# getreu/stringsext

Measured on AMD Instinct MI355X. Metric: GiB/s scanned, higher is better.
Workload: dtype u8

## Files before the change

### stringsext_amd/csrc/sx_device.hpp

```cpp
#pragma once
#include <cstdlib>
#include <hip/hip_runtime_api.h>
#include <stdint.h>

#include "../../include/stringsext_amd.h"

namespace sx {

constexpr uint32_t kTileBytes = 1024;

struct DevRun {
    uint64_t start;
    uint32_t len;
    uint32_t chars_flags;
};
constexpr uint32_t kRecStartOpen = 0x80000000u;
constexpr uint32_t kRecEndOpen = 0x40000000u;
constexpr uint32_t kRecCharsMask = 0x3FFFFFFFu;
constexpr uint32_t kRecInvalidLen = 0xFFFFFFFFu, kRecInvalidFlags = 0xFFFFFFFFu;

constexpr uint32_t kStatBase = 32, kStatShards = 16, kStatStride = 32, kCounterWords = kStatBase + kStatShards * kStatStride;

enum ClassifierKind : uint32_t {
    kClsSingleByteLut = 0,
// ... 76 lines not shown
struct ReplayRegionOut {
    uint64_t end;
    uint32_t n_find, n_bytes, status, pad;
};
size_t replay_heads_scratch_bytes(uint64_t n_runs);
hipError_t launch_replay_heads(const ReplayParams& P, uint32_t* slot_of, uint32_t* n_heads, uint32_t* head_list, ReplayRegionOut* ro,
                               void* scratch, size_t scratch_bytes,
                               hipStream_t stream);
hipError_t launch_replay_count(const ReplayParams& P, ReplayRegionOut* out, hipStream_t stream, int count_waves);
bool replay_fast_covers(const ReplayParams& P);
hipError_t launch_replay_fast(const ReplayParams& P, ReplayRegionOut* out, hipStream_t stream);
hipError_t launch_replay_write(const ReplayParams& P, const uint64_t* region_index, const uint64_t* fbase,
                               const uint64_t* abase, uint64_t n_regions, sx_finding* findings, uint8_t* arena,
                               hipStream_t stream);

size_t split_scratch_bytes(uint64_t n_runs);
hipError_t launch_split_count(const ReplayParams& P, void* scratch, size_t scratch_bytes, uint64_t* d_total, hipStream_t stream);
hipError_t launch_split_write(const ReplayParams& P, const void* scratch, uint64_t n_pieces, sx_run* out, hipStream_t stream);

inline uint32_t stitch_block_runs(uint64_t n_runs, int block_override) {
    if (block_override > 0) return (uint32_t)block_override;
    return n_runs > (1ull << 20) ? 512u : 128u;
}
enum : uint32_t { kTotEnd = 0, kTotLast, kTotFindings, kTotBytes, kTotStanding, kTotReplayBytes, kTotTooLong, kTotLastStart, kTotCount };
size_t stitch_scratch_bytes(uint64_t n_runs);
size_t stitch_blocks_bytes(uint64_t n_runs, int block_override);
hipError_t launch_stitch_blocks(const ReplayParams& P, const ReplayRegionOut* ro, uint8_t* stands, void* blocks,
                                uint64_t* totals, hipStream_t stream, int block_override);
hipError_t launch_stitch_finish(const ReplayParams& P, const ReplayRegionOut* ro, uint8_t* stands, const void* blocks,
                                uint64_t E0, uint64_t* fpos, uint64_t* apos, uint64_t* totals, void* scratch,
                                size_t scratch_bytes, hipStream_t stream, int block_override);
hipError_t launch_replay_write_flagged(const ReplayParams& P, const ReplayRegionOut* ro, const uint8_t* stands,
                                       const uint64_t* fpos, const uint64_t* apos, sx_finding* findings,
                                       uint8_t* arena, uint64_t avg_out_bytes, hipStream_t stream);

struct WvSwar {
    uint32_t cls;
    uint32_t n;
    uint32_t c1[6], c2[6], hi[6];
    uint32_t hi_len;
    uint32_t lr_c1[2], lr_c2[2];
    uint32_t kana;
};
struct WaveParams {
    const uint8_t* data;
    uint64_t len;
    uint64_t consumed0;
    uint32_t slice_base;
    uint32_t W, wps, q, n_min;
    uint64_t g_lo, g_hi;
    uint32_t nwin;
    uint32_t inject;
    int32_t mission_id, file_id;
    uint32_t family;
    const uint8_t* lut;
    const uint16_t* table;
    const uint32_t* pairs;
    uint32_t encoding;
    uint32_t entry_skip;
    uint32_t *wave_nf, *wave_nb, *wave_in, *wave_out;
    uint32_t* wave_grid;
    const uint64_t *wave_fbase, *wave_abase;
    uint64_t f_sub, a_sub;
    sx_finding* findings;
    uint8_t* arena;
    uint32_t packed;
    uint32_t str_off_base;
    uint64_t v0, v1;
    uint32_t* desc;
    uint32_t desc_cap;
    WvSwar swar;
    const uint32_t* pairs2;
    uint64_t* lead_set;
    uint64_t ubf;
    int32_t grep_char;
    uint32_t redo, use_entry;
    uint32_t same;
};
size_t wave_scratch_bytes(uint64_t n_waves);
hipError_t launch_wave_count(const WaveParams& P, uint64_t v0, uint64_t v1, uint64_t* fbase, uint64_t* abase, uint64_t* totals,
                             void* scratch, size_t scratch_bytes, hipStream_t stream);
hipError_t launch_wave_write(const WaveParams& P, uint64_t v0, uint64_t v1, hipStream_t stream);
hipError_t launch_wave_emit(const WaveParams& P, uint64_t v0, uint64_t v1, hipStream_t stream);

hipError_t merge_findings_device_part(const sx_finding* const* f, const uint8_t* const* a, const uint64_t* nf, const uint64_t* nb,
                                      const uint32_t* off0, int n_missions, void* out, void* scratch, size_t scratch_bytes,
                                      hipStream_t stream, int packed = 0, int ordered = 0);
bool merge_part_can_pack(uint64_t n, int n_missions);
hipError_t launch_slab_cuts(const ReplayParams& P, uint32_t n_slabs, uint64_t* idx, uint64_t* hi, hipStream_t stream);
hipError_t launch_merge_cuts(const sx_finding* f, uint64_t n, uint64_t nb, const uint64_t* cuts, uint32_t n_cuts, uint64_t* idx,
                             uint64_t* off, hipStream_t stream);
size_t merge_findings_scratch_bytes(uint64_t n_findings, int n_missions, int ordered = 0);
inline size_t up256(size_t v) { return (v + 255) / 256 * 256; }
size_t order_strings_scratch_bytes(uint64_t n);
hipError_t order_part_strings(void* recs, uint64_t n, int packed, const uint64_t* src, uint8_t* arena, void* scratch, size_t scratch_bytes,
                              hipStream_t stream);
struct PrintParams;
size_t print_scratch_bytes(uint64_t n);
hipError_t print_measure(const PrintParams& P, void* scratch, size_t scratch_bytes, hipStream_t stream, const uint64_t** wbase, const uint64_t** total);
hipError_t print_write(const PrintParams& P, hipStream_t stream);
struct SelectParams;
struct SelsetDevice;
struct SelreDevice;
struct LabelPick;
struct SelectBy {
    enum Kind { kPatterns, kSet, kRegex, kLabels } kind = kPatterns;
    union {
        const SelsetDevice* set = nullptr;
        const SelreDevice* re;
        const LabelPick* pick;
    };
};
size_t select_scratch_bytes(uint64_t n);
hipError_t selset_launch_match(const SelectParams& P, const SelsetDevice& set, uint64_t waves, hipStream_t stream);
hipError_t selre_launch_match(const SelectParams& P, const SelreDevice& re, uint64_t waves, hipStream_t stream);
hipError_t label_launch_pick(const SelectParams& P, const LabelPick& pick, uint64_t waves, hipStream_t stream);
hipError_t select_measure(SelectParams* P, const SelectBy& by, void* scratch, size_t scratch_bytes, hipStream_t stream, const uint32_t** count, const uint64_t** bytes);
size_t select_place_scratch_bytes(uint64_t n_sel);
hipError_t select_place(const SelectParams& P, void* out_recs, uint64_t n_sel, uint8_t* out_arena, void* scratch, size_t scratch_bytes, hipStream_t stream);
struct ExtractParams;
size_t extract_scratch_bytes(uint64_t n);
hipError_t extract_measure(ExtractParams* P, void* scratch, size_t scratch_bytes, hipStream_t stream, const uint64_t** count, const uint64_t** bytes);
size_t extract_place_scratch_bytes(uint64_t n_out);
hipError_t extract_place(const ExtractParams& P, void* out_recs, uint64_t n_out, uint8_t* out_arena, void* scratch, size_t scratch_bytes, hipStream_t stream);
struct SeltallyParams;
hipError_t seltally_launch(const SeltallyParams& P, hipStream_t stream);
struct LabelParams;
hipError_t label_launch(const LabelParams& P, hipStream_t stream);
hipError_t launch_copy_bytes(void* dst, const void* src, uint64_t bytes, uint32_t workgroups, hipStream_t stream, int threads, bool nontemporal);
hipError_t launch_small_copy(void* pinned_dst, const void* dev_src, size_t bytes, hipStream_t stream);

size_t sort_scratch_bytes(uint32_t n);
hipError_t sort_records(DevRun* recs, uint32_t n, uint64_t max_key, void* scratch, size_t scratch_bytes, hipStream_t stream, bool timing);

size_t compact_scratch_bytes(uint64_t n_regions);
hipError_t invalidate_region_slack(DevRun* recs, const uint32_t* counts, uint64_t n_regions, uint32_t region_cap, hipStream_t stream);
hipError_t compact_regions(const DevRun* recs, const uint32_t* counts, uint64_t n_regions, uint32_t region_cap, DevRun* out,
                           uint32_t* total, void* scratch, size_t scratch_bytes, hipStream_t stream);

size_t merge_scratch_bytes(uint32_t n);
hipError_t merge_sorted_records(const DevRun* recs, uint32_t n, uint64_t min_chars, void* scratch, size_t scratch_bytes,
                                sx_run* out, uint32_t* out_count, hipStream_t stream);

hipError_t launch_scan(ClassifierKind kind, const ScanParams& p, hipStream_t stream);
constexpr int kFusedMax = 3;
struct FusedParams {
    ScanParams m[kFusedMax];
    const uint8_t* data;
    uint64_t len;
    uint32_t subchunk;
    uint32_t fsh[kFusedMax][4];
    uint32_t cand_f[kFusedMax];
    uint32_t pf_zero[kFusedMax];
};
int fused_slot_of(ClassifierKind kind, const ScanParams& p);
hipError_t launch_scan_fused(const FusedParams& fp, uint32_t used, hipStream_t stream, int prefilter_override);
hipError_t launch_fill_background(uint8_t* dst, uint64_t first_index, uint64_t len, uint64_t seed,
                                  hipStream_t stream);
hipError_t launch_read_sum(const uint8_t* src, uint64_t len, uint64_t* out, hipStream_t stream, uint32_t subchunk = 0, uint32_t rot = 0);
hipError_t launch_gather(const uint8_t* src, uint8_t* dst, const uint64_t* seg_src, const uint64_t* seg_dst,
                         const uint32_t* seg_len, uint32_t n, hipStream_t stream);

}
```

### stringsext_amd/csrc/sx_fused.hip

```cpp
#include "sx_scan_core.hpp"

namespace sx {

struct NoCls {};

SX_DEV u32 shr1_keep(u32 v, u32 old) { return __builtin_amdgcn_update_dpp(old, v, 0x138, 0xF, 0xF, false); }
SX_DEV u32 ror1(u32 v) { return __builtin_amdgcn_mov_dpp(v, 0x13C, 0xF, 0xF, false); }

static_assert(offsetof(FusedParams, m) == 0, "late_params addresses m[slot] from the start of the kernel-argument segment");
typedef const __attribute__((address_space(4))) ScanParams* KArgMission;
SX_DEV KArgMission late_params(u32 slot) {
    asm volatile("" : "+s"(slot));
    return (KArgMission)__builtin_amdgcn_kernarg_segment_ptr() + slot;
}

struct LateEmitter {
    u32 slot, wave;
    u32 rcount, heavy_n;
    SX_DEV void append(bool want, u64 start, u64 end, u32 chars, u32 flags) {
        const u64 m = __ballot(want);
        if (m == 0) return;
        const KArgMission mp = late_params(slot);
        const u32 cap = mp->region_cap;
        DevRun* const recs = mp->recs;
        const u32 k = rcount + (u32)__popcll(m & ((1ull << lane_id()) - 1ull));
        rcount += (u32)__popcll(m);
        if (want && k < cap) {
            DevRun r;
            r.start = start;
            r.len = (u32)(end - start);
            r.chars_flags = (chars > kRecCharsMask ? kRecCharsMask : chars) | flags;
            recs[wave * cap + k] = r;
        }
    }
    SX_DEV void end_region() {
        const KArgMission mp = late_params(slot);
        const u32 cap = mp->region_cap;
        u32* const counters = mp->counters;
        u32* const shard = counters + kStatBase + (wave & (kStatShards - 1u)) * kStatStride;
        if (lane_id() == 0) {
            if (heavy_n) atomicAdd(shard, heavy_n);
            mp->region_counts[wave] = rcount < cap ? rcount : cap;
            if (rcount) atomicAdd(shard + 1, rcount);
            if (rcount > cap) {
                atomicAdd(counters, rcount - cap);
                atomicMax(counters + 3, rcount);
            }
        }
    }
};

template <class CLS>
struct Prefilter {
    static constexpr bool kHas = false;
    SX_DEV void init(u32) {}
    template <int MODE> SX_DEV bool hit(u32x4) const { return true; }
    SX_DEV bool last_unit_may_pass(u32, u32) const { return true; }
    static int mode_for(const ScanParams&) { return 0; }
    static u32 zero_bits(const ScanParams&) { return 0; }
};
template <int BE_T, int ODD_T>
struct Prefilter<Utf16RangeT<BE_T, ODD_T>> {
    static_assert(BE_T >= 0 && ODD_T >= 0, "the fused kernel knows byte order and parity at compile time");
    static constexpr bool kHas = true;
    u32 zz;
    static u32 zero_bits(const ScanParams& p) {
        u32 top = 0;
        if (p.a_lo <= p.a_hi) top = p.a_hi;
        if (p.u_lo <= p.u_hi && p.u_hi > top) top = p.u_hi;
        u32 mh = top >> 8;
        mh |= mh >> 1; mh |= mh >> 2; mh |= mh >> 4;
        return 0xFFu & ~mh;
    }
    SX_DEV void init(u32 z) { zz = (BE_T ^ ODD_T) ? z * 0x00010001u : z * 0x01000100u; }
    static int mode_for(const ScanParams& p) { return zero_bits(p) == 0u ? 0 : p.min_chars >= 7u ? 1 : p.min_chars >= 3u ? 2 : 0; }
    template <int MODE> SX_DEV bool hit(u32x4 x) const {
        if (MODE == 1) {
            const u32 q0 = __builtin_amdgcn_bitop3_b32(x.x, zz, x.y, 0xC8), q1 = __builtin_amdgcn_bitop3_b32(x.z, zz, x.w, 0xC8);
            return (q0 < q1 ? q0 : q1) == 0u;
        }
        const u32 a = x.x & zz, b = x.y & zz, c = x.z & zz, d = x.w & zz;
        const u32 ab = a < b ? a : b, cd = c < d ? c : d;
        return (ab < cd ? ab : cd) == 0u;
    }
    SX_DEV bool last_unit_may_pass(u32 prev_w, u32 cur_x) const {
        const u32 z8 = (zz | (zz >> 8)) & 0xFFu;
        const u32 hi = BE_T == ODD_T ? prev_w >> 24 : (BE_T ? prev_w >> 16 : cur_x);
        return (hi & z8) == 0u;
    }
};

template <class T, class = void> struct has_classify_g : std::false_type {};
template <class T> struct has_classify_g<T, std::void_t<decltype(std::declval<const T&>().classify_g(u32x4{}, 0u))>> : std::true_type {};
template <class CLS>
SX_DEV u32 classify_fast(const CLS& c, u32x4 x, u32 nx) {
    if constexpr (has_classify_g<CLS>::value) return c.classify_g(x, nx);
    else return c.template classify<false>(x, nx, 32u, false);
}

template <class T, class = void> struct has_starts_from_good : std::false_type {};
template <class T> struct has_starts_from_good<T, std::void_t<decltype(T::kStartsFromGood)>> : std::true_type {};

constexpr u32 kUnknown = 0x80000000u;

template <class CLS, int PFM, int SLOT>
struct Slot {
    static constexpr bool kUsed = !std::is_same<CLS, NoCls>::value;
    static constexpr u32 kSlot = SLOT;
    using PF = Prefilter<CLS>;
    static constexpr bool kPf = PFM != 0 && PF::kHas;
    static constexpr int kPfMode = PFM;
    CLS cls;
    PF pf;
    Carry c;
    LateEmitter em;
    u32 E;
    u32 gtmp, pgtmp, rtmp;
    u32 sh0, sh1, sh2, sh3;
};

template <class C0, class C1, class C2, int PFM>
__global__ __launch_bounds__(256) __attribute__((amdgpu_waves_per_eu(PFM ? 6 : 5))) void scan_kernel_fused(const FusedParams fp) {
    const u32 lane = lane_id();
    Slot<C0, PFM, 0> s0; Slot<C1, PFM, 1> s1; Slot<C2, PFM, 2> s2;

    const u32 wave = blockIdx.x * 4u + uniform(threadIdx.x >> 6);
    const u64 len = fp.len;
    const u64 sub_start = (u64)wave * (u64)fp.subchunk;
    if (sub_start >= len) return;
    const u64 sub_end = (sub_start + fp.subchunk < len) ? sub_start + fp.subchunk : len;

    auto make_cls = [&](auto& cls, u32 slot) {
        using CLS = std::decay_t<decltype(cls)>;
        if constexpr (!std::is_same<CLS, NoCls>::value) {
            const KArgMission mp = late_params(slot);
            ScanParams q;
            q.a_lo = mp->a_lo; q.a_hi = mp->a_hi; q.u_lo = mp->u_lo; q.u_hi = mp->u_hi; q.l3_lo = mp->l3_lo; q.l3_hi = mp->l3_hi;
            q.parity = mp->parity; q.big_endian = mp->big_endian; q.high_all = mp->high_all;
            cls.init(q, nullptr);
        }
    };
    auto setup = [&](auto& S) {
        using ST = std::decay_t<decltype(S)>;
        if constexpr (ST::kUsed) {
            constexpr u32 slot = ST::kSlot;
            if constexpr (ST::kPf) S.pf.init(fp.pf_zero[slot]);
            else make_cls(S.cls, slot);
            S.sh0 = fp.fsh[slot][0]; S.sh1 = fp.fsh[slot][1]; S.sh2 = fp.fsh[slot][2]; S.sh3 = fp.fsh[slot][3];
            S.em.slot = slot; S.em.wave = wave; S.em.rcount = 0; S.em.heavy_n = 0;
            S.c.g63 = 0; S.c.tracked = 0; S.c.t_chars = 0; S.c.t_flags = 0; S.c.t_start = 0;
            S.E = 0; S.gtmp = 0; S.pgtmp = 0; S.rtmp = 0;
        }
    };
    setup(s0); setup(s1); setup(s2);

    const bool has_pre = sub_start >= kTileBytes;
    const u64 win_lo = has_pre ? sub_start - kTileBytes : 0;
    u64 win_hi = sub_end + 2 * kTileBytes;
    if (win_hi > len) win_hi = len;
    const uint8_t* base_ptr = fp.data + win_lo;
    const u32 base_lo = uniform((u32)(uintptr_t)base_ptr), base_hi = uniform((u32)((uintptr_t)base_ptr >> 32));
    const __amdgpu_buffer_rsrc_t rsrc = __builtin_amdgcn_make_buffer_rsrc(
        (void*)(((u64)base_hi << 32) | base_lo), 0, (int)uniform(((u32)(win_hi - win_lo) + 15u) & ~15u), 0x00020000);
    auto load = [&](u32 off) -> u32x4 { return __builtin_amdgcn_raw_buffer_load_b128(rsrc, (int)off, 0, 0); };
    struct TileRegs { u32x4 d; u32 e; };
    auto fetch = [&](u32 off) -> TileRegs {
        TileRegs r;
        const u32 a = off + lane * 16u;
        r.d = load(a);
        r.e = __builtin_amdgcn_raw_buffer_load_b32(rsrc, (int)(a + 16u), 0, 0);
        return r;
    };

    const int n_tiles = (int)((sub_end - sub_start + kTileBytes - 1) / kTileBytes);
    int n_safe = n_tiles;
    while (n_safe > 0 && sub_start + (u64)n_safe * kTileBytes + 16 > len) n_safe--;

    int t = has_pre ? -1 : 0;
    u32 toff = 0;
    TileRegs R0 = fetch(0u), R1 = fetch(kTileBytes), R2;

    auto avail_at = [&](u64 tile_base) -> u32 {
        const u64 b = tile_base + 16ull * lane;
        return b >= len ? 0u : (len - b > 32 ? 32u : (u32)(len - b));
    };
    auto starts_before = [&](const auto& cls, u32 off, u64 tile_base) -> u32 {
        if (off < 16u) return 0u;
        asm volatile("" : "+s"(off));
        const u32x4 x = load(off - 16u);
        const u32 nx = __builtin_amdgcn_raw_buffer_load_b32(rsrc, (int)off, 0, 0);
        const u64 b = tile_base - 16;
        const u32 avail = b >= len ? 0u : (len - b > 32 ? 32u : (u32)(len - b));
        return uniform(cls.template classify<true>(x, nx, avail, true));
    };
    auto context_before = [&](const auto& cls, u32 off, u64 tile_base) -> u32 {
        if (off < kTileBytes) return 0u;
        u32 o = off - kTileBytes;
        asm volatile("" : "+s"(o));
        const TileRegs P = fetch(o);
        const u32 g = cls.template classify<false>(P.d, P.e, avail_at(tile_base - kTileBytes), true);
        const u32 pg = from_prev(g, 0u);
        const u32 gf = (g & 0xFFFFu) | (pg >> 16);
        return bcast(gf | (g & 0xFFFF0000u), 63);
    };

    auto generic_slot = [&](auto& S, const TileRegs& X, u64 tile_base, u32 avail, bool ne, bool have_g) {
        using ST = std::decay_t<decltype(S)>;
        if constexpr (ST::kUsed) {
            constexpr u32 slot = ST::kSlot;
            using CLS = std::decay_t<decltype(S.cls)>;
            CLS local;
            const CLS* cls = &S.cls;
            if constexpr (ST::kPf) {
                const u32 open = S.c.tracked | (S.c.g63 & 0x8000u) | ((S.c.g63 == kUnknown && t == 0) ? 1u : 0u);
                if (t < 0 || (__ballot(S.pf.template hit<ST::kPfMode>(X.d)) == 0 && open == 0u)) { S.c.g63 = kUnknown; return; }
                make_cls(local, slot);
                cls = &local;
                if (S.c.g63 == kUnknown) S.c.g63 = context_before(local, toff, tile_base);
            } else {
                S.c.g63 = bcast(have_g ? S.pgtmp : S.E, 0);
            }
            const KArgMission mp = late_params(slot);
            const u32x4 cur = X.d;
            const u32 g63_in = S.c.g63;
            const bool tracked_in = S.c.tracked != 0;
            const bool fast_g = have_g && !ST::kPf;
            const u32 g = fast_g ? S.gtmp : cls->template classify<false>(cur, X.e, avail, ne);
            const u32 pg = fast_g ? S.pgtmp : from_prev(g, g63_in);
            const u32 gf = (g & 0xFFFFu) | (pg >> 16);
            const u32 g63_out = bcast(gf | (g & 0xFFFF0000u), 63);
            u32 w = (g << 16) | pg;
            u32 r = w;
            if (fast_g) r = S.rtmp;
            else { r &= r << S.sh0; r &= r << S.sh1; r = r & (r << S.sh2) & (r << S.sh3); }
            const bool any_cand = __ballot((r & 0xFFFF0000u) != 0) != 0;
            const bool first_tile = t == 0;
            const bool first_open = first_tile && (g63_in & 0x8000u);
            if (t < 0 || (!any_cand && !tracked_in && !first_open)) {
                S.c.g63 = g63_out;
            } else {
                const u32 min_chars = mp->min_chars;
                const u64 lane_base = tile_base + 16ull * lane;
                u32 s;
                if constexpr (has_starts_from_good<CLS>::value) s = ne ? cls->template classify<true>(cur, X.e, avail, true) : cls->starts_from_good(cur, gf);
                else s = cls->template classify<true>(cur, X.e, avail, ne);
                w = (gf << 16) | (from_prev(gf, g63_in) & 0xFFFFu);
                const u32 s63 = (g63_in & 0x8000u) ? starts_before(*cls, toff, tile_base) : 0u;
                const u32 sw = (s << 16) | (from_prev(s, s63) & 0xFFFFu);
                bool done = false;
                if (!tracked_in && !first_open) done = light_path(w, sw, r, lane_base, S.em, min_chars);
                if (done) S.c.g63 = g63_out;
                else {
                    S.em.heavy_n++;
                    const u64 tile_end = tile_base + kTileBytes < sub_end ? tile_base + kTileBytes : sub_end;
                    heavy_path(gf, s, g, g63_in, s63, r >> 16, tile_base, tile_end, S.c, S.em, min_chars, fp.cand_f[slot], first_tile);
                }
            }
            if constexpr (!ST::kPf) S.E = S.c.g63;
        }
    };
    auto generic_tile = [&](const TileRegs& X, u32 which, bool have_g) {
        const u64 tile_base = sub_start + (u64)((long long)t * (long long)kTileBytes);
        const bool ne = t >= n_safe;
        const u32 avail = ne ? avail_at(tile_base) : 32u;
        if (which & 1u) generic_slot(s0, X, tile_base, avail, ne, have_g);
        if (which & 2u) generic_slot(s1, X, tile_base, avail, ne, have_g);
        if (which & 4u) generic_slot(s2, X, tile_base, avail, ne, have_g);
        toff += kTileBytes; t++;
    };

    auto fast_slot = [&](auto& S, const TileRegs& X, const TileRegs& Zp, bool zprev) -> bool {
        using ST = std::decay_t<decltype(S)>;
        if constexpr (!ST::kUsed) return true;
        else if constexpr (ST::kPf) {
            const u32 open = S.c.tracked | (S.c.g63 & 0x8000u);
            if ((__ballot(S.pf.template hit<ST::kPfMode>(X.d)) | (u64)open) != 0) {
                if (S.c.g63 == kUnknown && zprev && !S.pf.last_unit_may_pass(bcast(Zp.d.w, 63), bcast(X.d.x, 0))) S.c.g63 = 0;
                return false;
            }
            S.c.g63 = kUnknown;
            return true;
        } else {
            const u32 g = classify_fast(S.cls, X.d, X.e);
            const u32 pg = shr1_keep(g, S.E);
            const u32 w = (g << 16) | pg;
            u32 r = w;
            r &= r << S.sh0; r &= r << S.sh1; r = r & (r << S.sh2) & (r << S.sh3);
            S.gtmp = g; S.pgtmp = pg; S.rtmp = r;
            S.E = ror1(g);
            return (__ballot((r & 0xFFFF0000u) != 0) | (u64)S.c.tracked) == 0;
        }
    };
    auto fast_tile = [&](const TileRegs& X, TileRegs& Z, bool zprev) -> u32 {
        u32 zero = 0, one = 1, two = 2;
        asm volatile("" : "+s"(zero), "+s"(one), "+s"(two));
        u32 slow = fast_slot(s1, X, Z, zprev) ? zero : two;
        if (!fast_slot(s2, X, Z, zprev)) slow |= 4u;
        Z = fetch(toff + 2 * kTileBytes);
        slow |= fast_slot(s0, X, Z, false) ? zero : one;
        if (slow == 0) { toff += kTileBytes; t++; }
        return slow;
    };
    constexpr u32 kAll = (Slot<C0, PFM, 0>::kUsed ? 1u : 0u) | (Slot<C1, PFM, 1>::kUsed ? 2u : 0u) | (Slot<C2, PFM, 2>::kUsed ? 4u : 0u);

    for (;;) {
        while (t < n_tiles && (t <= 0 || t + 3 > n_safe)) {
            R2 = fetch(toff + 2 * kTileBytes);
            generic_tile(R0, kAll, false);
            R0 = R1; R1 = R2;
        }
        if (t >= n_tiles) break;
        bool zprev = false;
        do {
            u32 slow;
            if ((slow = fast_tile(R0, R2, zprev)) != 0) generic_tile(R0, slow, true);
            if ((slow = fast_tile(R1, R0, true)) != 0) generic_tile(R1, slow, true);
            if ((slow = fast_tile(R2, R1, true)) != 0) generic_tile(R2, slow, true);
            zprev = true;
        } while (t + 3 <= n_safe);
    }

    auto finish = [&](auto& S) {
        using ST = std::decay_t<decltype(S)>;
        if constexpr (ST::kUsed) {
            constexpr u32 slot = ST::kSlot;
            using CLS = std::decay_t<decltype(S.cls)>;
            const u64 after = sub_start + (u64)n_tiles * kTileBytes;
            CLS local;
            const CLS* cls = &S.cls;
            if constexpr (ST::kPf) {
                make_cls(local, slot);
                cls = &local;
                if (S.c.g63 == kUnknown) S.c.g63 = context_before(local, toff, after);
            } else S.c.g63 = bcast(S.E, 0);
            if (S.c.tracked || (S.c.g63 & 0x8000u)) {
                u64 os; u32 och, ofl;
                if (S.c.tracked) { os = S.c.t_start; och = S.c.t_chars; ofl = S.c.t_flags; }
                else {
                    const u32 suf = trailing_ones16(S.c.g63 & 0xFFFFu);
                    const u32 s63 = starts_before(*cls, toff, after);
                    os = after - suf;
                    och = (u32)__popc((s63 & 0xFFFFu) >> (16u - suf));
                    ofl = 0;
                }
                S.em.append(lane == 0, os, sub_end, och, ofl | kRecEndOpen);
            }
            S.em.end_region();
        }
    };
    finish(s0); finish(s1); finish(s2);
}

template <class C0, class C1, class C2>
static hipError_t launch_f(const FusedParams& fp, uint32_t used, hipStream_t stream, int prefilter_override) {
    const u64 waves = (fp.len + fp.subchunk - 1) / fp.subchunk;
    const u64 blocks = (waves + 3) / 4;
    if (blocks == 0) return hipSuccess;
    FusedParams q = fp;
    int mode = 1;
    if ((used & 2u) && Prefilter<C1>::mode_for(fp.m[1]) != 1) mode = Prefilter<C1>::mode_for(fp.m[1]);
    if ((used & 4u) && mode && Prefilter<C2>::mode_for(fp.m[2]) != 1) mode = Prefilter<C2>::mode_for(fp.m[2]) == 0 ? 0 : 2;
    if (!(used & 6u)) mode = 0;
    if (prefilter_override == 0) mode = 0; else if (prefilter_override == 2 && mode == 1) mode = 2;
    q.pf_zero[0] = 0; q.pf_zero[1] = Prefilter<C1>::zero_bits(fp.m[1]); q.pf_zero[2] = Prefilter<C2>::zero_bits(fp.m[2]);
    if (mode == 1) hipLaunchKernelGGL((scan_kernel_fused<C0, C1, C2, 1>), dim3((unsigned)blocks), dim3(256), 0, stream, q);
    else if (mode == 2) hipLaunchKernelGGL((scan_kernel_fused<C0, C1, C2, 2>), dim3((unsigned)blocks), dim3(256), 0, stream, q);
    else hipLaunchKernelGGL((scan_kernel_fused<C0, C1, C2, 0>), dim3((unsigned)blocks), dim3(256), 0, stream, q);
    return hipGetLastError();
}

int fused_slot_of(ClassifierKind kind, const ScanParams& p) {
    if (p.region_cap == 0 || p.persistent) return -1;
    if (kind == kClsUtf8Range2) return 0;
    if (kind == kClsUtf16Range) return p.big_endian ? 2 : 1;
    return -1;
}

hipError_t launch_scan_fused(const FusedParams& fp, uint32_t used, hipStream_t stream, int prefilter_override) {
    u32 parity = 0;
    if (used & 2u) parity = fp.m[1].parity & 1u; else if (used & 4u) parity = fp.m[2].parity & 1u;
    FusedParams q = fp;
    for (int s = 0; s < kFusedMax; s++) {
        if (!((used >> s) & 1u)) continue;
        q.data = fp.m[s].data; q.len = fp.m[s].len; q.subchunk = fp.m[s].subchunk;
        const u32 c = std::min<u32>(fp.m[s].cand_bytes, 12u);
        q.cand_f[s] = c;
        u32 have = 1;
        const u32 sh0 = have < c ? 1u : 0u; have += sh0;
        const u32 sh1 = have < c ? std::min(have, c - have) : 0u; have += sh1;
        const u32 rem = c - have;
        const u32 sh2 = std::min(have, rem), sh3 = rem;
        q.fsh[s][0] = sh0; q.fsh[s][1] = sh1; q.fsh[s][2] = sh2; q.fsh[s][3] = sh3;
    }
#define SX_ARG(...) __VA_ARGS__
#define SX_F(U, P, A, B, C) if (used == U && parity == P) return launch_f<A, B, C>(q, used, stream, prefilter_override);
    SX_F(1u, 0u, Utf8Range2, NoCls, NoCls)
    SX_F(7u, 0u, Utf8Range2, SX_ARG(Utf16RangeT<0, 0>), SX_ARG(Utf16RangeT<1, 0>))
    SX_F(7u, 1u, Utf8Range2, SX_ARG(Utf16RangeT<0, 1>), SX_ARG(Utf16RangeT<1, 1>))
    SX_F(3u, 0u, Utf8Range2, SX_ARG(Utf16RangeT<0, 0>), NoCls)
    SX_F(3u, 1u, Utf8Range2, SX_ARG(Utf16RangeT<0, 1>), NoCls)
    SX_F(5u, 0u, Utf8Range2, NoCls, SX_ARG(Utf16RangeT<1, 0>))
    SX_F(5u, 1u, Utf8Range2, NoCls, SX_ARG(Utf16RangeT<1, 1>))
    SX_F(6u, 0u, NoCls, SX_ARG(Utf16RangeT<0, 0>), SX_ARG(Utf16RangeT<1, 0>))
    SX_F(6u, 1u, NoCls, SX_ARG(Utf16RangeT<0, 1>), SX_ARG(Utf16RangeT<1, 1>))
#undef SX_F
#undef SX_ARG
    return hipErrorInvalidValue;
}

}
```

### stringsext_amd/csrc/sx_stage_a.cpp

```cpp
#include "sx_ctx.hpp"

using namespace sx;

namespace sx {

static bool large_regions_fit(uint64_t len, uint64_t n_regions, uint32_t cap) {
    const uint64_t slots = n_regions * cap;
    return slots < (1ull << 31) && slots * sizeof(DevRun) <= std::max<uint64_t>(256ull << 20, len / 2);
}

static uint32_t subchunk_bytes(const sx_ctx* ctx) {
    const uint32_t sub = ctx->opt.subchunk_bytes ? ctx->opt.subchunk_bytes : 256u * 1024u;
    return std::max<uint32_t>(kTileBytes, sub / kTileBytes * kTileBytes);
}

static bool fusion_allowed(const sx_ctx* ctx) {
    return !(ctx->opt.flags & (SX_OPT_NO_FUSED_SCAN | SX_OPT_MISSION_STREAMS)) && !ctx->sw.mission_streams && ctx->sw.fused && ctx->sw.scan_warm < 0;
}

ScanParams scan_params(const sx_ctx* ctx, int mission, const ScanSlot& s, const uint8_t* d_bytes, uint64_t len,
                       uint32_t parity, uint64_t min_chars) {
    const Mission& m = ctx->missions[(size_t)mission];
    ScanParams p = m.proto;
    p.data = d_bytes; p.len = len; p.subchunk = subchunk_bytes(ctx); p.parity = parity;
    p.pair_lut = ctx->dev[(size_t)mission].d_pair_lut;
    if (p.gb4) {
        p.gb_ranges = ctx->dev[(size_t)mission].d_table ? ctx->dev[(size_t)mission].d_table + kGbN : nullptr;
        p.ubf = m.c.ubf;
        if (!p.gb_ranges) p.gb4 = 0;
    }
    p.wave_prio = ctx->sw.scan_prio;
    p.min_chars = (uint32_t)std::min<uint64_t>(min_chars, kRecCharsMask);
    if (p.min_chars == 0) p.min_chars = 1;
    p.cand_bytes = std::min<uint32_t>(p.min_chars * (m.is_utf16() ? 2u : 1u), 14u);
    {
        uint32_t have = 1;
        for (int i = 0; i < 5; i++) {
            const uint32_t sh = have < p.cand_bytes ? std::min(have, p.cand_bytes - have) : 0;
            p.cand_sh[i] = sh;
            have += sh;
        }
    }
    p.capacity = s.capacity; p.recs = s.d_recs; p.counters = s.d_counters;
    p.region_cap = s.region_cap; p.region_counts = s.d_cnt; p.grid_flags = s.d_grid;
    unsigned occ = ctx->scan_blocks_per_cu;
    p.persistent = (occ >= 1 && occ < 8) ? occ * ctx->n_cus : 0u;
    return p;
}

int stage_a_launch(sx_ctx* ctx, const std::vector<int>& which, const uint8_t* d_bytes, uint64_t len,
                   const std::vector<uint32_t>& parity, const std::vector<uint64_t>& min_chars, int si) {
    if (len == 0) return SX_OK;
    for (size_t k = 0; k < which.size(); k++) {
        MissionDev& d = ctx->dev[(size_t)which[k]];
        ScanSlot& s = d.slot[si];
        if (s.free_pending) { HIP_TRY(ctx, hipStreamWaitEvent(d.stream, s.ev_free, 0)); s.free_pending = false; }
        {
            const uint32_t sub = subchunk_bytes(ctx);
            const uint64_t n_regions = (len + sub - 1) / sub;
            if (ctx->dense.size() != ctx->missions.size()) ctx->dense.assign(ctx->missions.size(), 0);
            s.region_cap = 0; s.n_regions = n_regions;
            const uint32_t dn = ctx->dense[(size_t)which[k]];
            const uint32_t want_cap = dn > 1 ? dn : (dn == 0 ? ctx->region_cap : 0u);
            if (ctx->region_cap && want_cap &&
                (dn > 1 ? large_regions_fit(len, n_regions, want_cap) : n_regions * want_cap < (1ull << 28))) {
                s.region_cap = want_cap;
                int rc = ensure_capacity(ctx, s, (uint32_t)(n_regions * s.region_cap));
                if (rc != SX_OK && dn > 1) {
                    (void)hipGetLastError();
                    ctx->dense[(size_t)which[k]] = 1;
                    s.region_cap = 0;
                    rc = SX_OK;
                }
                if (rc != SX_OK) return rc;
                if (s.region_cap == 0) goto launch;
                if (s.cnt_cap < n_regions) {
                    if (s.d_cnt) HIP_TRY(ctx, hipFree(s.d_cnt));
                    s.d_cnt = nullptr; s.cnt_cap = 0;
                    HIP_TRY(ctx, hipMalloc((void**)&s.d_cnt, (n_regions + n_regions / 4 + 64) * 4));
                    s.cnt_cap = n_regions + n_regions / 4 + 64;
                }
            }
        }
    launch:
        const bool dbcs = ctx->missions[(size_t)which[k]].is_dbcs();
        if (dbcs) {
            const uint32_t sub = subchunk_bytes(ctx);
            const uint64_t n_sub = (len + sub - 1) / sub;
            if (s.grid_cap < n_sub) {
                if (s.d_grid) HIP_TRY(ctx, hipFree(s.d_grid));
                s.d_grid = nullptr; s.grid_cap = 0;
                HIP_TRY(ctx, hipMalloc((void**)&s.d_grid, (n_sub + n_sub / 4 + 64) * 4));
                s.grid_cap = n_sub + n_sub / 4 + 64;
            }
        }
    }
    std::vector<char> fused(which.size(), 0);
    std::vector<ScanParams> params(which.size());
    for (size_t k = 0; k < which.size(); k++)
        params[k] = scan_params(ctx, which[k], ctx->dev[(size_t)which[k]].slot[si], d_bytes, len, parity[k], min_chars[k]);
    if (fusion_allowed(ctx)) {
        FusedParams fp{};
        uint32_t used = 0;
        size_t member[kFusedMax] = { 0, 0, 0 };
        for (size_t k = 0; k < which.size(); k++) {
            if (params[k].persistent) continue;
            const int sl = fused_slot_of(ctx->missions[(size_t)which[k]].kind, params[k]);
            if (sl < 0 || (used >> sl) & 1u) continue;
            if (sl >= 1 && (used & 6u) && ((fp.m[(used & 2u) ? 1 : 2].parity ^ params[k].parity) & 1u)) continue;
            used |= 1u << sl; fp.m[sl] = params[k]; member[sl] = k;
        }
        if (__builtin_popcount(used) >= 2 || used == 1u) {
            hipStream_t st = nullptr;
            for (int sl = 0; sl < kFusedMax; sl++) if ((used >> sl) & 1u) {
                MissionDev& d = ctx->dev[(size_t)which[member[sl]]];
                if (!st) st = d.stream;
                HIP_TRY(ctx, hipMemsetAsync(d.slot[si].d_counters, 0, kCounterWords * sizeof(uint32_t), st));
            }
            for (int sl = 0; sl < kFusedMax; sl++) if ((used >> sl) & 1u) HIP_TRY(ctx, hipEventRecord(ctx->dev[(size_t)which[member[sl]]].slot[si].ev0, st));
            HIP_TRY(ctx, launch_scan_fused(fp, used, st, ctx->sw.fused_prefilter));
            bool first = true;
            for (int sl = 0; sl < kFusedMax; sl++) if ((used >> sl) & 1u) {
                ScanSlot& s = ctx->dev[(size_t)which[member[sl]]].slot[si];
                HIP_TRY(ctx, hipEventRecord(s.ev1, st));
                s.fused = true; s.fused_first = first; first = false;
                fused[member[sl]] = 1;
            }
            ctx->stats.fused_launches++;
        }
    }
    for (size_t k = 0; k < which.size(); k++) {
        if (fused[k]) continue;
        MissionDev& d = ctx->dev[(size_t)which[k]];
        ScanSlot& s = d.slot[si];
        s.fused = false; s.fused_first = false;
        const bool dbcs = ctx->missions[(size_t)which[k]].is_dbcs();
        const ScanParams& p = params[k];
        const uint64_t n_sub = (len + p.subchunk - 1) / p.subchunk;
        for (int w = ctx->sw.scan_warm; w > 0; w--) {
            if (dbcs) HIP_TRY(ctx, hipMemsetAsync(s.d_grid, 0, n_sub * 4, d.stream));
            HIP_TRY(ctx, hipMemsetAsync(s.d_counters, 0, kCounterWords * sizeof(uint32_t), d.stream));
            HIP_TRY(ctx, launch_scan(ctx->missions[(size_t)which[k]].kind, p, d.stream));
        }
        if (dbcs) HIP_TRY(ctx, hipMemsetAsync(s.d_grid, 0, n_sub * 4, d.stream));
        HIP_TRY(ctx, hipMemsetAsync(s.d_counters, 0, kCounterWords * sizeof(uint32_t), d.stream));
        HIP_TRY(ctx, hipEventRecord(s.ev0, d.stream));
        HIP_TRY(ctx, launch_scan(ctx->missions[(size_t)which[k]].kind, p, d.stream));
        HIP_TRY(ctx, hipEventRecord(s.ev1, d.stream));
        if (dbcs) { d.grid_of_scan = s.d_grid; d.grid_sub = p.subchunk; d.grid_data = d_bytes; d.grid_len = len; }
    }
    return SX_OK;
}

int stage_a_finish(sx_ctx* ctx, const std::vector<int>& which, const uint8_t* d_bytes, uint64_t len,
                   const std::vector<uint32_t>& parity, const std::vector<uint64_t>& min_chars, int si,
                   std::vector<RunList>* out, bool cut_into_pieces, const ReplayJob* wave_job) {
    out->assign(which.size(), RunList{});
    if (len == 0) return SX_OK;
    const double t0 = now_ms();
    for (size_t k = 0; k < which.size(); k++) {
        MissionDev& d = ctx->dev[(size_t)which[k]];
        ScanSlot& s = d.slot[si];
        HIP_TRY(ctx, hipEventSynchronize(s.ev1));
        const double t_ev = now_ms();
        SX_TL("mission %d: scan kernel done", which[k]);
        float ms = 0;
        HIP_TRY(ctx, hipEventElapsedTime(&ms, s.ev0, s.ev1));
        if (which[k] < 16) ctx->stats.kernel_ms[which[k]] += ms;
        if (s.fused && s.fused_first) ctx->stats.fused_ms += ms;
        if (which[k] < 64) { if (s.fused) ctx->stats.fused_mask |= 1ull << which[k]; else ctx->stats.fused_mask &= ~(1ull << which[k]); }
        uint32_t counters[4] = { 0, 0, 0, 0 };
        std::vector<uint32_t> hc(kCounterWords);
        bool skip_runs = false;
        for (int round = 0;; round++) {
            { const int rb = read_back_sync(ctx, d, d.stream_b, hc.data(), s.d_counters, kCounterWords * sizeof(uint32_t)); if (rb != SX_OK) return rb; }
            counters[0] = hc[0]; counters[3] = hc[3];
            {
                uint64_t heavy = 0, recs = 0;
                for (uint32_t sh = 0; sh < kStatShards; sh++) { heavy += hc[kStatBase + sh * kStatStride]; recs += hc[kStatBase + sh * kStatStride + 1]; }
                counters[1] = (uint32_t)std::min<uint64_t>(heavy, 0xFFFFFFFFull); counters[2] = (uint32_t)std::min<uint64_t>(recs, 0xFFFFFFFFull);
            }
            if (round == 0 && wave_job) {
                const uint64_t total = s.region_cap ? counters[2] : counters[0];
                if (wave_replay_wanted(ctx, *wave_job, (size_t)which[k], total, counters[1])) {
                    RunList& rl = (*out)[k];
                    rl.n = wave_replay_wanted(ctx, *wave_job, (size_t)which[k], total) ? total : std::max<uint64_t>(total, len / 16);
                    rl.p = nullptr; rl.skipped = true; rl.complete = true;
                    skip_runs = true;
                    break;
                }
            }
            if (s.region_cap) {
                if (counters[0] == 0) break;
                const uint32_t big = (counters[3] + counters[3] / 4 + 127) / 64 * 64;
                if (s.region_cap == ctx->region_cap && counters[3] && large_regions_fit(len, s.n_regions, big) && !ctx->sw.no_large_regions) {
                    ctx->dense[(size_t)which[k]] = big;
                    s.region_cap = big;
                    if (ensure_capacity(ctx, s, (uint32_t)(s.n_regions * big)) != SX_OK) {
                        (void)hipGetLastError();
                        ctx->dense[(size_t)which[k]] = 1;
                        s.region_cap = 0;
                    }
                } else {
                    ctx->dense[(size_t)which[k]] = 1;
                    s.region_cap = 0;
                }
            } else {
                if (counters[0] <= s.capacity) break;
                if (round >= 8) { ctx->err = "device run-record buffer kept overflowing"; return SX_E_NOMEM; }
                int rc = ensure_capacity(ctx, s, counters[0] + counters[0] / 8 + 1024);
                if (rc != SX_OK) return rc;
            }
            const ScanParams p = scan_params(ctx, which[k], s, d_bytes, len, parity[k], min_chars[k]);
            const double tr0 = now_ms();
            if (p.grid_flags) HIP_TRY(ctx, hipMemsetAsync(p.grid_flags, 0, ((len + p.subchunk - 1) / p.subchunk) * 4, d.stream_b));
            HIP_TRY(ctx, hipMemsetAsync(s.d_counters, 0, kCounterWords * sizeof(uint32_t), d.stream_b));
            HIP_TRY(ctx, launch_scan(ctx->missions[(size_t)which[k]].kind, p, d.stream_b));
            if (p.grid_flags) { d.grid_of_scan = p.grid_flags; d.grid_sub = p.subchunk; d.grid_data = d_bytes; d.grid_len = len; }
            HIP_TRY(ctx, hipStreamSynchronize(d.stream_b));
            ctx->stats.rescans++;
            ctx->stats.rescan_ms += now_ms() - tr0;
        }
        const double tc0 = now_ms();
        SX_TL("mission %d: counters read (%u records)", which[k], s.region_cap ? counters[2] : counters[0]);
        if (ctx->sw.timing2) fprintf(stderr, "[sx]   mission %d: kernel done at +%.2f ms, counters at +%.2f ms\n", which[k], t_ev - t0, tc0 - t0);
        if (skip_runs) {
            HIP_TRY(ctx, hipEventRecord(s.ev_free, d.stream_b));
            s.free_pending = true;
            if (ctx->sw.timing) fprintf(stderr, "[sx] mission %d: kernel %.2f ms, %llu records counted: string-dense, every window is replayed\n", which[k], ms, (unsigned long long)(*out)[k].n);
            ctx->stats.run_records += (*out)[k].n;
            ctx->stats.bytes_scanned += len;
            ctx->stats.heavy_tiles += counters[1];
            continue;
        }
        uint32_t nrec = counters[0];
        const DevRun* d_records = s.d_recs;
        const bool large_regions = s.region_cap > ctx->region_cap && ctx->region_cap;
        const bool regions = s.region_cap != 0 && !large_regions;
        if (large_regions) {
            HIP_TRY(ctx, invalidate_region_slack(s.d_recs, s.d_cnt, s.n_regions, s.region_cap, d.stream_b));
            nrec = (uint32_t)(s.n_regions * s.region_cap);
        }
        if (regions) {
            const uint64_t slots = s.n_regions * s.region_cap;
            if (s.packed_cap < slots) {
                if (s.d_packed) HIP_TRY(ctx, hipFree(s.d_packed));
                s.d_packed = nullptr; s.packed_cap = 0;
                HIP_TRY(ctx, hipMalloc((void**)&s.d_packed, (slots + slots / 8 + 64) * sizeof(DevRun)));
                s.packed_cap = slots + slots / 8 + 64;
            }
            int rc = ensure_scratch(ctx, compact_scratch_bytes(s.n_regions)); if (rc != SX_OK) return rc;
            HIP_TRY(ctx, compact_regions(s.d_recs, s.d_cnt, s.n_regions, s.region_cap, s.d_packed, s.d_counters + 1, ctx->d_scratch,
                                         ctx->d_scratch_cap, d.stream_b));
            { const int rb = read_back_sync(ctx, d, d.stream_b, &nrec, s.d_counters + 1, 4); if (rb != SX_OK) return rb; }
            d_records = s.d_packed;
            SX_TL("mission %d: regions packed (%u)", which[k], nrec);
        } else if (ctx->region_cap && !large_regions && nrec < s.n_regions * ctx->region_cap / 4)
            ctx->dense[(size_t)which[k]] = 0;
        const uint32_t join_min = ctx->sw.device_join_min;
        const bool dev_sorted = nrec >= join_min && nrec > 0;
        double tc1 = tc0;
        RunList& rl = (*out)[k];
        if (dev_sorted) {
            const size_t sb = std::max(sort_scratch_bytes(nrec), merge_scratch_bytes(nrec));
            int rc = ensure_scratch(ctx, sb); if (rc != SX_OK) return rc;
            if (d.ev_runs) HIP_TRY(ctx, hipEventSynchronize(d.ev_runs));
            rc = ensure_rp(ctx, d, 0, (uint64_t)nrec * sizeof(sx_run)); if (rc != SX_OK) return rc;
            if (!regions) HIP_TRY(ctx, sort_records(s.d_recs, nrec, len, ctx->d_scratch, ctx->d_scratch_cap, d.stream_b, ctx->sw.timing2));
            if (ctx->sw.timing2) { HIP_TRY(ctx, hipStreamSynchronize(d.stream_b)); fprintf(stderr, "[sx]   sort done +%.2f ms\n", now_ms() - tc0); }
            HIP_TRY(ctx, merge_sorted_records(d_records, nrec, min_chars[k], ctx->d_scratch, ctx->d_scratch_cap,
                                              (sx_run*)d.d_rp[0], s.d_counters + 2, d.stream_b));
            HIP_TRY(ctx, hipEventRecord(s.ev_free, d.stream_b));
            s.free_pending = true;
// ... 77 lines not shown
```

### stringsext_amd/csrc/sx_switches.cpp

```cpp
#include "sx_switches.hpp"

#include <stdio.h>
#include <stdlib.h>

#include <algorithm>

namespace sx {

static bool present(const char* name) { return getenv(name) != nullptr; }
static bool on_unless_0(const char* name) { const char* e = getenv(name); return !(e && !atoi(e)); }
static bool on_if_nonzero(const char* name) { const char* e = getenv(name); return e && atoi(e); }
static int int_or(const char* name, int unset) { const char* e = getenv(name); return e ? atoi(e) : unset; }
static int64_t i64_or(const char* name, int64_t unset) { const char* e = getenv(name); return e ? (int64_t)atoll(e) : unset; }
static int clamped_or(const char* name, int lo, int hi, int unset) { const char* e = getenv(name); return e ? std::max(lo, std::min(hi, atoi(e))) : unset; }
static uint64_t u64_at_least(const char* name, uint64_t lo, uint64_t unset) { const char* e = getenv(name); return e ? std::max<uint64_t>(lo, (uint64_t)atoll(e)) : unset; }

Switches Switches::from_env() {
    Switches s;
    if (const char* e = getenv("SX_PIN_FLAGS")) s.pin_flags = (int64_t)(unsigned)strtoul(e, nullptr, 0);
    s.small_copy = on_unless_0("SX_SMALL_COPY");
    if (const char* e = getenv("SX_REPLAY_THREADS")) s.replay_threads = (int)std::max(1u, std::min(256u, (unsigned)atoi(e)));
    s.result_on_device = on_if_nonzero("SX_RESULT_ON_DEVICE");
    s.scan_blocks_per_cu = int_or("SX_SCAN_BLOCKS_PER_CU", s.scan_blocks_per_cu);
    if (const char* e = getenv("SX_REGION_CAP")) s.region_cap = (int64_t)(uint32_t)atoi(e);
    s.scan_cus = clamped_or("SX_SCAN_CUS", 1, INT32_MAX, s.scan_cus);
    if (const char* e = getenv("SX_PRIO")) s.prio_n = std::max(0, sscanf(e, "%d,%d", &s.prio_scan, &s.prio_post));
    s.mission_streams = present("SX_MISSION_STREAMS");
    s.scan_prio = (uint32_t)int_or("SX_SCAN_PRIO", (int)s.scan_prio);
    s.fused = on_unless_0("SX_FUSED");
    s.fused_prefilter = int_or("SX_FUSED_PREFILTER", s.fused_prefilter);
    s.scan_warm = clamped_or("SX_SCAN_WARM", 0, INT32_MAX, s.scan_warm);
    s.no_large_regions = present("SX_NO_LARGE_REGIONS");
    s.device_join_min = (uint32_t)int_or("SX_DEVICE_JOIN_MIN", (int)s.device_join_min);
    s.no_pieces = present("SX_NO_PIECES");
    s.probe_rot = (uint32_t)int_or("SX_PROBE_ROT", (int)s.probe_rot);
    s.host_replay = present("SX_HOST_REPLAY");
    s.device_replay = present("SX_DEVICE_REPLAY");
    s.host_stitch = present("SX_HOST_STITCH");
    s.no_replay_skip = present("SX_NO_REPLAY_SKIP");
    s.no_grid_bound = present("SX_NO_GRID_BOUND");
    s.no_replay_cache = present("SX_NO_REPLAY_CACHE");
    s.max_region_windows = (uint32_t)clamped_or("SX_MAX_REGION_WINDOWS", 1, INT32_MAX, (int)s.max_region_windows);
    s.replay_cache_mib = i64_or("SX_REPLAY_CACHE_MIB", s.replay_cache_mib);
    s.fast_replay = on_unless_0("SX_FAST_REPLAY");
    s.count_waves = int_or("SX_COUNT_WAVES", s.count_waves);
    s.stitch_block = clamped_or("SX_STITCH_BLOCK", 0, INT32_MAX, s.stitch_block);
    s.slabs = clamped_or("SX_SLABS", 1, 64, s.slabs);
    s.replay_copy_wgs = int_or("SX_REPLAY_COPY_WGS", s.replay_copy_wgs);
    s.host_merge = present("SX_HOST_MERGE");
    s.packed = on_unless_0("SX_PACKED");
    s.merge_part_mib = u64_at_least("SX_MERGE_PART_MIB", 1, s.merge_part_mib);
    s.merge_part_findings = u64_at_least("SX_MERGE_PART_FINDINGS", 1024, s.merge_part_findings);
    s.merge_copy_wgs = int_or("SX_MERGE_COPY_WGS", s.merge_copy_wgs);
    s.merge_copy_nt = int_or("SX_MERGE_COPY_NT", s.merge_copy_nt);
    s.merge_copy_threads = clamped_or("SX_MERGE_COPY_THREADS", 64, 1024, s.merge_copy_threads);
    s.host_merge_seg_bytes = u64_at_least("SX_HOST_MERGE_SEG_BYTES", 1, s.host_merge_seg_bytes);
    s.splice_seg_bytes = u64_at_least("SX_SPLICE_SEG_BYTES", 1, s.splice_seg_bytes);
    s.piece_mib = i64_or("SX_PIECE_MIB", s.piece_mib);
    s.seq_piece_kib = i64_or("SX_SEQ_PIECE_KIB", s.seq_piece_kib);
    s.seq_piece_mib = i64_or("SX_SEQ_PIECE_MIB", s.seq_piece_mib);
    s.debug_entry = present("SX_DEBUG_ENTRY");
    s.busiest_last = int_or("SX_BUSIEST_LAST", s.busiest_last);
    if (const char* e = getenv("SX_DEFER_MIN_BYTES")) s.defer_min_bytes = (uint64_t)atoll(e);
    s.wave_threads = on_unless_0("SX_WAVE_THREADS");
    s.timeline = int_or("SX_TIMELINE", s.timeline);
    s.timing = present("SX_TIMING");
    s.timing2 = present("SX_TIMING2");
    if (const char* e = getenv("SX_WAVE_REPLAY")) s.wave_replay = atoi(e) != 0;
    s.wave_keep_scan = present("SX_WAVE_KEEP_SCAN");
    if (const char* e = getenv("SX_WAVE_BYTES_PER_RUN")) s.wave_bytes_per_run = (uint64_t)atoll(e);
    s.wave_stream_prio = int_or("SX_WAVE_STREAM_PRIO", s.wave_stream_prio);
    s.wave_batches = clamped_or("SX_WAVE_BATCHES", 1, 64, s.wave_batches);
    s.wave_slabs = clamped_or("SX_WAVE_SLABS", 1, 64, s.wave_slabs);
    s.wave_lut = on_if_nonzero("SX_WAVE_LUT");
    s.wave_desc = on_unless_0("SX_WAVE_DESC");
    s.wave_desc_cap = clamped_or("SX_WAVE_DESC_CAP", 1, INT32_MAX, s.wave_desc_cap);
    s.wave_fail = present("SX_WAVE_FAIL");
    if (const char* e = getenv("SX_WAVE_REPAIR")) s.wave_repair = atoi(e) ? std::max(1, atoi(e)) : 0;
    s.wave_same = on_unless_0("SX_WAVE_SAME");
    if (const char* e = getenv("SX_SCAN_STREAM_MIB")) s.scan_stream_mib = (uint64_t)atoll(e);
    s.ingest_mmap = present("SX_INGEST_MMAP");
    return s;
}

}
```

### stringsext_amd/csrc/sx_switches.hpp

```cpp
#pragma once
#include <stdint.h>

namespace sx {

struct Switches {
    int64_t pin_flags = -1;
    bool small_copy = true;
    int replay_threads = 0;
    bool result_on_device = false;
    int scan_blocks_per_cu = -1;
    int64_t region_cap = -1;
    int scan_cus = 0;
    int prio_n = -1, prio_scan = 0, prio_post = 0;
    bool mission_streams = false;
    uint32_t scan_prio = 0;
    bool fused = true;
    int fused_prefilter = -1;
    int scan_warm = -1;
    bool no_large_regions = false;
    uint32_t device_join_min = 65536;
    bool no_pieces = false;
    uint32_t probe_rot = 0;
    bool host_replay = false;
    bool device_replay = false;
    bool host_stitch = false;
    bool no_replay_skip = false;
    bool no_grid_bound = false;
    bool no_replay_cache = false;
    uint32_t max_region_windows = 0;
    int64_t replay_cache_mib = -1;
    bool fast_replay = true;
    int count_waves = 4;
    int stitch_block = 0;
    int slabs = 0;
    int replay_copy_wgs = 0;
    bool host_merge = false;
    bool packed = true;
    uint64_t merge_part_mib = 0;
    uint64_t merge_part_findings = 0;
    int merge_copy_wgs = -1;
    int merge_copy_nt = 1;
    int merge_copy_threads = 512;
    uint64_t host_merge_seg_bytes = 0;
    uint64_t splice_seg_bytes = 0;
    int64_t piece_mib = -1;
    int64_t seq_piece_kib = -1;
    int64_t seq_piece_mib = -1;
    bool debug_entry = false;
    int busiest_last = 0;
    uint64_t defer_min_bytes = 256ull << 20;
    bool wave_threads = true;
    int timeline = 0;
    bool timing = false;
    bool timing2 = false;
    int wave_replay = -1;
    bool wave_keep_scan = false;
    uint64_t wave_bytes_per_run = 0;
    int wave_stream_prio = -1;
    int wave_batches = 0;
    int wave_slabs = 0;
    bool wave_lut = false;
    bool wave_desc = true;
    int wave_desc_cap = 0;
    bool wave_fail = false;
    int wave_repair = -1;
    bool wave_same = true;
    uint64_t scan_stream_mib = 0;
    bool ingest_mmap = false;

    static Switches from_env();
};

}
```

Measured before the change: 4091.

## Add scalar lone-lane fast path for fused scan tiles with one flagged lane

When a tile in the fused scanner has no tracked run and exactly one lane holds candidate run bits, the slot's classification state is broadcast to scalar values and resolved by a new lone_resolve routine. That routine emits the records directly, skipping the full wave-wide shift/reach and emit pipeline. It is gated by template forms that exclude some classifier combinations and by a runtime flag in the kernel arguments, on by default. The new branch adds code, extra ballots and broadcasts, and register pressure to the fused kernel, and it duplicates the emission logic.

Result: no change. 4108 (median of 6 runs) (+0.4%).

```diff
diff --git a/stringsext_amd/csrc/sx_device.hpp b/stringsext_amd/csrc/sx_device.hpp
--- a/stringsext_amd/csrc/sx_device.hpp
+++ b/stringsext_amd/csrc/sx_device.hpp
@@ -252,9 +252,10 @@
     uint32_t fsh[kFusedMax][4];
     uint32_t cand_f[kFusedMax];
     uint32_t pf_zero[kFusedMax];
+    uint32_t lone;
 };
 int fused_slot_of(ClassifierKind kind, const ScanParams& p);
-hipError_t launch_scan_fused(const FusedParams& fp, uint32_t used, hipStream_t stream, int prefilter_override);
+hipError_t launch_scan_fused(const FusedParams& fp, uint32_t used, hipStream_t stream, int prefilter_override, bool lone);
 hipError_t launch_fill_background(uint8_t* dst, uint64_t first_index, uint64_t len, uint64_t seed,
                                   hipStream_t stream);
 hipError_t launch_read_sum(const uint8_t* src, uint64_t len, uint64_t* out, hipStream_t stream, uint32_t subchunk = 0, uint32_t rot = 0);
diff --git a/stringsext_amd/csrc/sx_fused.hip b/stringsext_amd/csrc/sx_fused.hip
--- a/stringsext_amd/csrc/sx_fused.hip
+++ b/stringsext_amd/csrc/sx_fused.hip
@@ -1,4 +1,6 @@
 #include "sx_scan_core.hpp"
+#define SXD __device__ __forceinline__
+#include "sx_lone_core.hpp"
 
 namespace sx {
 
@@ -12,6 +14,10 @@
 SX_DEV KArgMission late_params(u32 slot) {
     asm volatile("" : "+s"(slot));
     return (KArgMission)__builtin_amdgcn_kernarg_segment_ptr() + slot;
+}
+SX_DEV u32 late_word(u32 off) {
+    asm volatile("" : "+s"(off));
+    return *(const __attribute__((address_space(4))) u32*)((const __attribute__((address_space(4))) char*)__builtin_amdgcn_kernarg_segment_ptr() + off);
 }
 
 struct LateEmitter {
@@ -101,6 +107,11 @@
 template <class T, class = void> struct has_starts_from_good : std::false_type {};
 template <class T> struct has_starts_from_good<T, std::void_t<decltype(T::kStartsFromGood)>> : std::true_type {};
 
+template <class C0, class C1, class C2, int PFM> struct LoneForm { static constexpr bool value = true; };
+template <int PFM> struct LoneForm<Utf8Range2, Utf16RangeT<0, 1>, NoCls, PFM> { static constexpr bool value = PFM == 0; };
+template <> struct LoneForm<Utf8Range2, Utf16RangeT<0, 0>, NoCls, 0> { static constexpr bool value = false; };
+template <> struct LoneForm<Utf8Range2, NoCls, Utf16RangeT<1, 0>, 0> { static constexpr bool value = false; };
+
 constexpr u32 kUnknown = 0x80000000u;
 
 template <class CLS, int PFM, int SLOT>
@@ -218,6 +229,41 @@
                 cls = &local;
                 if (S.c.g63 == kUnknown) S.c.g63 = context_before(local, toff, tile_base);
             } else {
+                if constexpr (LoneForm<C0, C1, C2, PFM>::value && has_starts_from_good<CLS>::value) if (have_g && S.c.tracked == 0) {
+                    const u64 flagged = __ballot((S.rtmp & 0xFFFF0000u) != 0);
+                    if (__popcll(flagged) == 1 && late_word((u32)offsetof(FusedParams, lone)) != 0u) {
+                        const u32 L = (u32)__builtin_ctzll(flagged);
+                        const u32 Lp = L ? L - 1u : 0u, Ln = L < 63u ? L + 1u : 63u;
+                        LoneIn in;
+                        in.own = bcast(S.gtmp, L);
+                        in.p1 = bcast(S.pgtmp, L);
+                        in.p2 = L ? bcast(S.pgtmp, Lp) : 0u;
+                        in.next = bcast(S.gtmp, Ln);
+                        in.first_lane = L == 0u; in.last_lane = L == 63u;
+                        in.bytes_prev[0] = bcast(X.d.x, Lp); in.bytes_prev[1] = bcast(X.d.y, Lp); in.bytes_prev[2] = bcast(X.d.z, Lp); in.bytes_prev[3] = bcast(X.d.w, Lp);
+                        in.bytes_own[0] = bcast(X.d.x, L); in.bytes_own[1] = bcast(X.d.y, L); in.bytes_own[2] = bcast(X.d.z, L); in.bytes_own[3] = bcast(X.d.w, L);
+                        const KArgMission lp = late_params(slot);
+                        const bool mine = lone_resolve(in, tile_base + 16ull * L, lp->min_chars, late_word((u32)offsetof(FusedParams, cand_f) + 4u * slot),
+                                                       [&](u64 start, u64 end, u32 chars) {
+                            const u32 cap = lp->region_cap;
+                            const u32 k = S.em.rcount;
+                            S.em.rcount = k + 1u;
+                            if (k < cap && lane == L) {
+                                DevRun rec;
+                                rec.start = start;
+                                rec.len = (u32)(end - start);
+                                rec.chars_flags = chars > kRecCharsMask ? kRecCharsMask : chars;
+                                lp->recs[S.em.wave * cap + k] = rec;
+                            }
+                        });
+                        if (mine) {
+                            const u32 g63 = bcast(S.gtmp, 63);
+                            S.c.g63 = (g63 & 0xFFFFu) | (bcast(S.pgtmp, 63) >> 16) | (g63 & 0xFFFF0000u);
+                            S.E = S.c.g63;
+                            return;
+                        }
+                    }
+                }
                 S.c.g63 = bcast(have_g ? S.pgtmp : S.E, 0);
             }
             const KArgMission mp = late_params(slot);
@@ -376,10 +422,11 @@
     return -1;
 }
 
-hipError_t launch_scan_fused(const FusedParams& fp, uint32_t used, hipStream_t stream, int prefilter_override) {
+hipError_t launch_scan_fused(const FusedParams& fp, uint32_t used, hipStream_t stream, int prefilter_override, bool lone) {
     u32 parity = 0;
     if (used & 2u) parity = fp.m[1].parity & 1u; else if (used & 4u) parity = fp.m[2].parity & 1u;
     FusedParams q = fp;
+    q.lone = lone ? 1u : 0u;
     for (int s = 0; s < kFusedMax; s++) {
         if (!((used >> s) & 1u)) continue;
         q.data = fp.m[s].data; q.len = fp.m[s].len; q.subchunk = fp.m[s].subchunk;
diff --git a/stringsext_amd/csrc/sx_lone_core.hpp b/stringsext_amd/csrc/sx_lone_core.hpp
--- /dev/null
+++ b/stringsext_amd/csrc/sx_lone_core.hpp
@@ -0,0 +1,68 @@
+#pragma once
+#include <stdint.h>
+
+#ifndef SXD
+#define SXD inline
+#endif
+
+namespace sx {
+
+struct LoneIn {
+    uint32_t own;
+    uint32_t p1;
+    uint32_t p2;
+    uint32_t next;
+    uint32_t first_lane;
+    uint32_t last_lane;
+    uint32_t bytes_prev[4];
+    uint32_t bytes_own[4];
+};
+
+SXD uint32_t lone_cont4(uint32_t v) {
+    const uint32_t f = (v & ~(v << 1) & 0x80808080u) >> 7;
+    return ((f * 0x00204081u) >> 21) & 0xFu;
+}
+SXD uint32_t lone_cont16(const uint32_t d[4]) { return lone_cont4(d[0]) | (lone_cont4(d[1]) << 4) | (lone_cont4(d[2]) << 8) | (lone_cont4(d[3]) << 12); }
+
+SXD uint32_t lone_reach(uint32_t w, uint32_t cand_f) {
+    uint32_t r = w, have = 1;
+    while (have < cand_f) {
+        const uint32_t step = have < cand_f - have ? have : cand_f - have;
+        r &= r << step;
+        have += step;
+    }
+    return r;
+}
+
+template <class EMIT>
+SXD bool lone_resolve(const LoneIn& in, uint64_t lane_base, uint32_t min_chars, uint32_t cand_f, EMIT&& emit) {
+    if (in.first_lane && (in.p1 & 0x8000u)) return false;
+    const uint32_t gf = (in.own & 0xFFFFu) | (in.p1 >> 16);
+    const uint32_t gp = ((in.p1 & 0xFFFFu) | (in.p2 >> 16)) & 0xFFFFu;
+    const uint32_t w = (gf << 16) | gp;
+    const uint32_t s_own = gf & ~lone_cont16(in.bytes_own) & 0xFFFFu;
+    const uint32_t s_prev = in.first_lane ? 0u : gp & ~lone_cont16(in.bytes_prev);
+    const uint32_t sw = (s_own << 16) | s_prev;
+    const uint32_t r = lone_reach(w, cand_f);
+    const uint32_t n0 = in.last_lane ? 1u : ((in.next | (in.own >> 16)) & 1u);
+    const uint32_t g16 = gf & 0xFFFFu;
+    const uint32_t ends = g16 & ~((g16 >> 1) | (n0 << 15));
+    uint32_t cand = ends & (r >> 16);
+    if (in.last_lane && (r >> 31)) return false;
+    if (cand) {
+        const uint32_t e0 = 16u + (uint32_t)__builtin_ctz(cand);
+        if (((~w) & ((1u << e0) - 1u)) == 0u) return false;
+    }
+    while (cand) {
+        const uint32_t e = 16u + (uint32_t)__builtin_ctz(cand);
+        const uint32_t below = (~w) & ((1u << e) - 1u);
+        const uint32_t st = 32u - (uint32_t)__builtin_clz(below);
+        const uint32_t field = (e >= 31u ? 0xFFFFFFFFu : ((1u << (e + 1u)) - 1u)) & ~((1u << st) - 1u);
+        const uint32_t ch = (uint32_t)__builtin_popcount(sw & field);
+        if (ch >= min_chars) emit(lane_base - 16 + st, lane_base - 16 + e + 1, ch);
+        cand &= cand - 1u;
+    }
+    return true;
+}
+
+}
diff --git a/stringsext_amd/csrc/sx_stage_a.cpp b/stringsext_amd/csrc/sx_stage_a.cpp
--- a/stringsext_amd/csrc/sx_stage_a.cpp
+++ b/stringsext_amd/csrc/sx_stage_a.cpp
@@ -118,7 +118,7 @@
                 HIP_TRY(ctx, hipMemsetAsync(d.slot[si].d_counters, 0, kCounterWords * sizeof(uint32_t), st));
             }
             for (int sl = 0; sl < kFusedMax; sl++) if ((used >> sl) & 1u) HIP_TRY(ctx, hipEventRecord(ctx->dev[(size_t)which[member[sl]]].slot[si].ev0, st));
-            HIP_TRY(ctx, launch_scan_fused(fp, used, st, ctx->sw.fused_prefilter));
+            HIP_TRY(ctx, launch_scan_fused(fp, used, st, ctx->sw.fused_prefilter, ctx->sw.fused_lone));
             bool first = true;
             for (int sl = 0; sl < kFusedMax; sl++) if ((used >> sl) & 1u) {
                 ScanSlot& s = ctx->dev[(size_t)which[member[sl]]].slot[si];
diff --git a/stringsext_amd/csrc/sx_switches.cpp b/stringsext_amd/csrc/sx_switches.cpp
--- a/stringsext_amd/csrc/sx_switches.cpp
+++ b/stringsext_amd/csrc/sx_switches.cpp
@@ -29,6 +29,7 @@
     s.scan_prio = (uint32_t)int_or("SX_SCAN_PRIO", (int)s.scan_prio);
     s.fused = on_unless_0("SX_FUSED");
     s.fused_prefilter = int_or("SX_FUSED_PREFILTER", s.fused_prefilter);
+    s.fused_lone = on_unless_0("SX_FUSED_LONE");
     s.scan_warm = clamped_or("SX_SCAN_WARM", 0, INT32_MAX, s.scan_warm);
     s.no_large_regions = present("SX_NO_LARGE_REGIONS");
     s.device_join_min = (uint32_t)int_or("SX_DEVICE_JOIN_MIN", (int)s.device_join_min);
diff --git a/stringsext_amd/csrc/sx_switches.hpp b/stringsext_amd/csrc/sx_switches.hpp
--- a/stringsext_amd/csrc/sx_switches.hpp
+++ b/stringsext_amd/csrc/sx_switches.hpp
@@ -16,6 +16,7 @@
     uint32_t scan_prio = 0;
     bool fused = true;
     int fused_prefilter = -1;
+    bool fused_lone = true;
     int scan_warm = -1;
     bool no_large_regions = false;
     uint32_t device_join_min = 65536;
```
